# gregorgebhardt/gym-kilobots

Hardware: AMD Instinct MI355X
Metric: kilobot-steps/sec (higher is better)
Workload: dtype f32

## Files before the change

gym_kilobots_amd/csrc/kb_regsolve_bins.inc:

```
{
    constexpr int KRB = KB_KREG_BINS;
    const bool solving = (int)__builtin_amdgcn_readfirstlane(wave) < nsolve;
    unsigned ra[KRB], rb[KRB], rm[KRB];
    float racc[KRB], rnx[KRB], rny[KRB];
    const unsigned WOFF = 8u * (unsigned)(NB - 5);
    char *const velB = reinterpret_cast<char *>(vel), *const posB = reinterpret_cast<char *>(pos);
#define RB_WALL(j) (ra[j] >= WOFF)
#define RB_WALLIDX(j) ((int)((ra[j] - WOFF) >> 3))
#define RB_VEL(off) (*reinterpret_cast<float2 *>(velB + (off)))
#define RB_POS(off) (*reinterpret_cast<float2 *>(posB + (off)))
#define RB_C(j) ((int)(rm[j] & 0xFFFu))
#define RB_DEPTH(j) ((int)((rm[j] >> 12) & 0x1FFu))
#define RB_FLIP(j) (((rm[j] >> 21) & 1u) != 0u)
#define RB_ISL(j) ((int)(rm[j] >> 22))
#pragma unroll
    for (int j = 0; j < KRB; ++j) { ra[j] = 0u; rb[j] = 0u; rm[j] = 0u; racc[j] = 0.0f; rnx[j] = 1.0f; rny[j] = 0.0f; }
    unsigned long long slotLevels[KRB];
    int dlo[KRB], dhi[KRB];
#pragma unroll
    for (int j = 0; j < KRB; ++j) { slotLevels[j] = 0ull; dlo[j] = 1; dhi[j] = 0; }
    int maxD = 0;
    unsigned mycnt = 0;
    const float nm_bb = p.nm_bb, nm_wb = p.nm_wb;
#ifdef KB_SOLVER_PRIO
// ... 173 lines not shown
                ra[j] = wallA ? WOFF + 8u * (unsigned)(a - WALL_CODE) : 8u * (unsigned)a;
                rb[j] = 8u * (unsigned)b;
                racc[j] = v_[j] ? acc_[j] : 0.0f;
                rm[j] = v_[j] ? (c_[j] | ((unsigned)rdepth[j] << 12) | (flip ? 1u << 21 : 0u) | (root_[j] << 22)) : 0u;
                float dist;
                wall_geom(p, wallA ? a - WALL_CODE : 0, pb_[j].x, pb_[j].y, dist, wnx[j], wny[j]);
                if (flip) { wnx[j] = -wnx[j]; wny[j] = -wny[j]; }
                dx[j] = pb_[j].x - pa_[j].x; dy[j] = pb_[j].y - pa_[j].y;
                dd[j] = dx[j] * dx[j] + dy[j] * dy[j];
                pairOn[j] = v_[j] && !wallA && dd[j] > B2_EPSILON * B2_EPSILON;
                ieee = ieee || (pairOn[j] && !kb_exact_guard(dd[j]));
                if (wallA) { rnx[j] = wnx[j]; rny[j] = wny[j]; } else { rnx[j] = 1.0f; rny[j] = 0.0f; }
            }
            if (__builtin_expect(__builtin_amdgcn_ballot_w64(ieee) == 0ull, 1)) {
#pragma unroll
                for (int j = 0; j < KRB; ++j) {
                    const float len = kb_sqrt_refine(dd[j], __builtin_amdgcn_sqrtf(dd[j]), __builtin_amdgcn_rsqf(dd[j]));
                    const float inv = kb_rcp_refine(len, __builtin_amdgcn_rcpf(len));
                    if (pairOn[j]) { rnx[j] = dx[j] * inv; rny[j] = dy[j] * inv; }
                }
            } else {
#pragma unroll
                for (int j = 0; j < KRB; ++j) {
                    const float len = sqrtf(dd[j]);
                    const float inv = 1.0f / len;
                    if (pairOn[j]) { rnx[j] = dx[j] * inv; rny[j] = dy[j] * inv; }
                }
            }
        }
#undef RB_A
#undef RB_B
#ifdef KB_PROFILE
        if (lane == 0) atomicMax(&misc[M_PROF], (unsigned)maxD);
        if (tid == 0) atomicAdd(&KB_PROF(M_PROF_DEPTH), (unsigned)maxD);
        KB_STAMP(7);
#endif
    }
    KB_ABLATE_EXIT(9);
#define RB_ON(j) (RB_DEPTH(j) == d_)
    if (solving) {
#pragma unroll
        for (int j = 0; j < KRB; ++j) {
            for (int d_ = dlo[j]; d_ <= dhi[j]; ++d_) {
                if (RB_ON(j)) {
                    const float2 va = RB_VEL(ra[j]), vb = RB_VEL(rb[j]);
                    const float Px = racc[j] * rnx[j], Py = racc[j] * rny[j];
                    const float ima = RB_WALL(j) ? 0.0f : p.im_bot;
                    RB_VEL(ra[j]) = make_float2(va.x - ima * Px, va.y - ima * Py);
                    RB_VEL(rb[j]) = make_float2(vb.x + p.im_bot * Px, vb.y + p.im_bot * Py);
                }
                wave_sync();
            }
        }
        KB_STAMP_PRE(29);
    }
    KB_ABLATE_EXIT(10);
    if (solving) {
        for (int it = 0; it < p.vel_iters; ++it) {
#pragma unroll
            for (int j = 0; j < KRB; ++j) {
                for (int d_ = dlo[j]; d_ <= dhi[j]; ++d_) {
                    if (RB_ON(j)) {
                        const float2 va = RB_VEL(ra[j]), vb = RB_VEL(rb[j]);
                        const bool wallA = RB_WALL(j);
                        const float nx = rnx[j], ny = rny[j];
                        const float ima = wallA ? 0.0f : p.im_bot, imb = p.im_bot;
                        const float dvx = vb.x - va.x, dvy = vb.y - va.y;
                        const float vn = dvx * nx + dvy * ny;
                        float lambda = -((wallA ? nm_wb : nm_bb) * vn);
                        const float accOld = racc[j];
                        const float newimp = fmaxf(accOld + lambda, 0.0f);
                        lambda = newimp - accOld;
                        racc[j] = newimp;
                        const float Px = lambda * nx, Py = lambda * ny;
                        RB_VEL(ra[j]) = make_float2(va.x - ima * Px, va.y - ima * Py);
                        RB_VEL(rb[j]) = make_float2(vb.x + imb * Px, vb.y + imb * Py);
                    }
                    wave_sync();
                }
            }
        }
        KB_STAMP_PRE(30);
    }
#ifdef KB_SOLVER_PRIO
    __builtin_amdgcn_s_setprio(0);
#endif
    __syncthreads();
    KB_STAMP(4);
    KB_RETID();
    KB_ABLATE_EXIT(11);
#ifdef KB_PROFILE
    if (tid == 0) atomicAdd(&KB_PROF(9), misc[M_PROF]);
#endif
    if (solving) {
#pragma unroll
        for (int j = 0; j < KRB; ++j)
            if (lane + 64u * j < mycnt) lAcc[RB_C(j)] = racc[j];
    }
#pragma unroll
    for (int q = 0; q < BPT; ++q) {
        const int b_ = tid + q * nt;
        if (b_ >= N) continue;
        const int b = ms[q];
        float vxx = vel[b].x, vyy = vel[b].y, ww = bw[q];
        startX[b] = pos[b].x; startY[b] = pos[b].y;
        const float tx = h * vxx, ty = h * vyy;
        if (tx * tx + ty * ty > B2_MAX_TRANSLATION_SQ) {
            const float ratio = B2_MAX_TRANSLATION / sqrtf(tx * tx + ty * ty);
            vxx *= ratio; vyy *= ratio;
        }
        const float rot = h * ww;
        if (rot * rot > B2_MAX_ROTATION_SQ) {
            const float ratio = B2_MAX_ROTATION / fabsf(rot);
            ww *= ratio;
        }
        pos[b].x += h * vxx; pos[b].y += h * vyy;
        th[q] += h * ww;
        vel[b].x = vxx; vel[b].y = vyy; bw[q] = ww;
        if (SLEEP) islWave[b] = (unsigned char)((active[b] ? 2 : 0) | (p.pos_iters <= 0 ? 1 : 0));
    }
    __syncthreads();
    KB_STAMP(5);
    KB_RETID();
    KB_ABLATE_EXIT(12);
    if (solving) {
#ifdef KB_SOLVER_PRIO
        __builtin_amdgcn_s_setprio(KB_SOLVER_PRIO);
#endif
        for (int it = 0; it < p.pos_iters; ++it) {
            unsigned char *act = active + (it & 1) * NB, *nxt = active + ((it + 1) & 1) * NB;
            bool viol = false;
            bool ron[KRB];
#pragma unroll
            for (int j = 0; j < KRB; ++j) ron[j] = (lane + 64u * j < mycnt) && act[RB_ISL(j)] != 0;
#pragma unroll
            for (int j = 0; j < KRB; ++j) {
                for (int d_ = dlo[j]; d_ <= dhi[j]; ++d_) {
                    if (ron[j] && RB_ON(j)) {
                    const bool wallA = RB_WALL(j);
                    const int isl = RB_ISL(j);
                    float nx, ny, sep;
                    const float ima = wallA ? 0.0f : p.im_bot, imb = p.im_bot;
                    const float2 pb = RB_POS(rb[j]);
                    const float bx = pb.x, by = pb.y;
                    float axx = 0.0f, ayy = 0.0f;
                    if (wallA) {
                        float dist, wx, wy;
                        wall_geom(p, RB_WALLIDX(j), bx, by, dist, wx, wy);
                        nx = RB_FLIP(j) ? -wx : wx; ny = RB_FLIP(j) ? -wy : wy;
                        const float along = RB_FLIP(j) ? -dist : dist;
                        sep = along - B2_POLYGON_RADIUS - p.r_bot;
                    } else {
                        const float2 pa = RB_POS(ra[j]);
                        axx = pa.x; ayy = pa.y;
                        const float dx = bx - axx, dy = by - ayy;
                        const float dd = dx * dx + dy * dy;
                        if (__builtin_expect(__builtin_amdgcn_ballot_w64(!kb_exact_guard(dd)) == 0ull, 1)) {
                            const float len = kb_sqrt_refine(dd, __builtin_amdgcn_sqrtf(dd), __builtin_amdgcn_rsqf(dd));
                            const float inv = kb_rcp_refine(len, __builtin_amdgcn_rcpf(len));
                            nx = dx * inv; ny = dy * inv;
                        } else {
                            const float len = sqrtf(dd);
                            nx = dx; ny = dy;
                            if (!(len < B2_EPSILON)) { const float inv = 1.0f / len; nx = dx * inv; ny = dy * inv; }
                        }
                        sep = (dx * nx + dy * ny) - p.r_bot - p.r_bot;
                    }
                    if (sep < -3.0f * B2_LINEAR_SLOP) { nxt[isl] = 1; viol = true; if (SLEEP && it == p.pos_iters - 1) islWave[isl] = 3; }
                    const float C = kb_clampf(B2_BAUMGARTE * (sep + B2_LINEAR_SLOP), -B2_MAX_LINEAR_CORRECTION, 0.0f);
                    const float K = ima + imb;
                    const float imp = __builtin_expect(p.exact_div, 1) ? kb_div_const(-C, K, wallA ? p.y_wb : p.y_bb) : (K > 0.0f ? -C / K : 0.0f);
                    const float Px = imp * nx, Py = imp * ny;
                    if (!wallA) RB_POS(ra[j]) = make_float2(axx - ima * Px, ayy - ima * Py);
                    RB_POS(rb[j]) = make_float2(bx + imb * Px, by + imb * Py);
                    }
                    wave_sync();
                }
            }
#ifdef KB_PROFILE
            if (tid == 0) atomicAdd(&KB_PROF(10), 1u);
#endif
            if (!__any(viol)) break;
#pragma unroll
            for (int j = 0; j < KRB; ++j) if (lane + 64u * j < mycnt) act[RB_ISL(j)] = 0;
            wave_sync();
        }
        KB_STAMP_PRE(24);
#ifdef KB_SOLVER_PRIO
        __builtin_amdgcn_s_setprio(0);
#endif
    }
#undef RB_WALL
#undef RB_WALLIDX
#undef RB_VEL
#undef RB_POS
#undef RB_C
#undef RB_DEPTH
#undef RB_FLIP
#undef RB_ISL
#undef RB_ON
}
```

gym_kilobots_amd/csrc/kb_step_kernel.h:

```cpp
#pragma once
#include <utility>

#include "kb_common.h"
#include "kb_objects.h"

namespace kb {

template <int DRIVE_MODE, int LIGHT_TYPE, bool OBJ, int FN = 0, int TIER = 0, bool POLY = true, bool SENSE = true, bool SLEEP = false>
__global__ void __launch_bounds__(TIER == 1 ? 64 : 64 * KB_MAX_WAVES, (TIER == 1 || TIER == 3) ? 2 : ((TIER == 2 || (FN != 0 && !OBJ)) ? KB_COMPACT_WAVES_PER_SIMD : KB_MIN_WAVES_PER_SIMD)) kb_step_kernel(const Params p) {
    constexpr bool WIDE = TIER == 1 || TIER == 3;
    constexpr bool BINS = !OBJ;
    constexpr int KRX = BINS ? KB_KREG_BINS : KREG;
    constexpr bool PAR_DS = FN != 0 && BINS;
    static_assert(!SLEEP || FN == 0 || !OBJ, "the fixed-size instantiations with objects do not carry the sleep state");
    extern __shared__ __align__(16) unsigned char smem[];
    int e = blockIdx.x;
    int tid = threadIdx.x;
    const int nt = FN ? 64 * KB_MAX_WAVES : (int)blockDim.x;
    int lane = tid & 63, wave = tid >> 6;
    const int wave_s = __builtin_amdgcn_readfirstlane(wave);
    const int nw = nt >> 6;
    const int nsolve = BINS ? (nw >= KB_NSOLVE_DIV ? nw / KB_NSOLVE_DIV : 1) : nw;
    const int N = FN ? FN : p.N, NP = FN ? ((FN + 3) & ~3) : p.NP, S = p.S;
    size_t o = (size_t)e * N;
    size_t wo = (size_t)e * p.cap;
    const float h = p.h;

    const int NB = FN ? ((FN + 3) & ~3) + KB_MAX_OBJECTS + 4 : p.NB;
    const int capL_ = (BINS && FN != 0) ? ldsb::CAPL : p.capL;
    const bool hashed = FN == 0 && p.hmask != 0;
    const int fx = lds::fixed(OBJ || FN != 0, nw), ot_ = lds::objtab(nw);
    float2 *pos = (float2 *)(smem + (BINS ? ldsb::pos() : lds::body32(fx, NB, 0))), *vel = (float2 *)(smem + (BINS ? ldsb::vel(NB) : lds::body32(fx, NB, 2)));
    float2 *start = (float2 *)(smem + lds::body32(fx, NB, 4));
    unsigned *dirCnt = (unsigned *)(smem + (BINS ? ldsb::dircnt(NB) : lds::body32(fx, NB, 6))), *parent = (unsigned *)(smem + (BINS ? ldsb::parent(NB) : lds::body32(fx, NB, 7)));
    unsigned *islCnt = dirCnt;
    unsigned *lPair = (unsigned *)(smem + (BINS ? ldsb::con32(NB, NP, hashed, capL_, 0) : lds::con32(fx, NB, capL_, 0))), *lInfo = (unsigned *)(smem + (BINS ? ldsb::con32(NB, NP, hashed, capL_, 1) : lds::con32(fx, NB, capL_, 1)));
    float *lAcc = (float *)(smem + (BINS ? ldsb::con32(NB, NP, hashed, capL_, 2) : lds::con32(fx, NB, capL_, 2)));
    float *oldAcc = (float *)(smem + (BINS ? ldsb::oldacc(NB, NP, hashed, capL_) : lds::con32(fx, NB, capL_, 3)));
    unsigned short *lCbk = (unsigned short *)(smem + (BINS ? ldsb::cbk(NB, NP, hashed, capL_) : lds::con16(fx, NB, capL_, 0)));
    unsigned short *lOrder = (unsigned short *)(smem + (BINS ? ldsb::order(NB, NP, hashed, capL_) : lds::con16(fx, NB, capL_, 1)));
    unsigned short *oldKey = (unsigned short *)(smem + (BINS ? ldsb::oldkey(NB, NP, hashed, capL_) : lds::con16(fx, NB, capL_, 2)));
    unsigned short *wsOff = (unsigned short *)(smem + (BINS ? ldsb::wsoff(NB) : lds::bot16(fx, NB, capL_, NP, 0))), *newOff = (unsigned short *)(smem + (BINS ? ldsb::newoff(NB, NP, hashed) : lds::bot16(fx, NB, capL_, NP, 1)));
    unsigned short *nextb = (unsigned short *)(smem + lds::bot16(fx, NB, capL_, NP, 2)), *cellOf = (unsigned short *)(smem + lds::bot16(fx, NB, capL_, NP, 3));
    unsigned char *wsCnt = smem + (BINS ? ldsb::wscnt(NB, NP) : lds::bot8(fx, NB, capL_, NP, 0)), *wsCntNew = smem + (BINS ? ldsb::wscntnew(NB, NP, hashed) : lds::bot8(fx, NB, capL_, NP, 1));
    unsigned char *active = smem + (BINS ? ldsb::act0(NB, NP, hashed, capL_) : lds::active(fx, NB, capL_, NP));
    unsigned char *islWave = smem + (BINS ? ldsb::islwave(NB, NP, hashed, capL_) : lds::islwave(fx, NB, capL_, NP));
    unsigned short *head = (unsigned short *)(smem + lds::head(fx, NB, capL_, NP));
    unsigned short *idOf = (unsigned short *)(smem + ldsb::idof(NB, NP)), *cellOfSlot = (unsigned short *)(smem + ldsb::cellofslot(NB, NP));
    unsigned short *E1 = (unsigned short *)(smem + ldsb::binE(NB, NP, hashed, capL_));
    unsigned short *tmpSort = reinterpret_cast<unsigned short *>(lInfo);
    float *startX = reinterpret_cast<float *>(smem + ldsb::botA(NB)), *startY = reinterpret_cast<float *>(dirCnt);
    unsigned *misc = (unsigned *)(smem + lds::MISC), *wsum = (unsigned *)(smem + lds::WSUM);
    const int tb_ = BINS ? ldsb::binE(NB, NP, hashed, capL_) - lds::BKSTART : 0;
    unsigned *bkStart = (unsigned *)(smem + tb_ + lds::BKSTART), *bkFill = (unsigned *)(smem + tb_ + lds::bkfill(nw));
    unsigned *bkMaxRank = (unsigned *)(smem + tb_ + lds::bkmaxrank(nw));
    unsigned short *bkList = (unsigned short *)(smem + tb_ + lds::bklist(nw));
    unsigned char *nList = smem + tb_ + lds::nlist(nw);
    float *objTab = (float *)(smem + ot_);
    float *objBody = (float *)(smem + ot_ + lds::OBJBODY);
    unsigned *objCnt = (unsigned *)(smem + ot_ + lds::OBJCNT);
    unsigned short *objList = (unsigned short *)(smem + ot_ + lds::OBJLIST);
    float *objW = (float *)(smem + ot_ + lds::OBJW), *objA = (float *)(smem + ot_ + lds::OBJA), *objA0 = (float *)(smem + ot_ + lds::OBJA0);
    unsigned long long *mcMask = (unsigned long long *)(smem + ot_ + lds::MCMASK);
    float *objSlp = (float *)(smem + ot_ + lds::OBJSLP);
    const int M = OBJ ? p.M : 0;
    constexpr bool MIX = DRIVE_MODE == KB_DRIVE_MIXED;
    static_assert(!MIX || (OBJ && FN == 0), "mixed drive laws run on the generic code path with per-body masses");
    unsigned char *botLaw = smem + (MIX ? p.botlaw_off : 0);
#define KB_IM_BOT(a_) (MIX ? p.im_mode[botLaw[a_]] : p.im_bot)
    auto bim = [&](int id) __attribute__((always_inline)) -> float {
        return id >= WALL_CODE ? 0.0f : ((!OBJ || id < N) ? KB_IM_BOT(id) : objBody[(id - N) * BT_WORDS + BT_IM]);
    };
    auto brad = [&](int id) __attribute__((always_inline)) -> float {
        return id >= WALL_CODE ? B2_POLYGON_RADIUS : ((!OBJ || id < N) ? p.r_bot : objBody[(id - N) * BT_WORDS + BT_RADIUS]);
    };
    auto bpoly = [&](int id) __attribute__((always_inline)) -> bool {
        return OBJ && POLY && id >= N && id < WALL_CODE && objBody[(id - N) * BT_WORDS + BT_KIND] != 0.0f;
    };
    ObjCtx ox;
    ox.pos = pos; ox.vel = vel; ox.objW = objW; ox.objA = objA; ox.objTab = objTab; ox.objBody = objBody;
    ox.mc = (float *)(smem + lds::mcarea(fx, NB, capL_, NP, p.nhead));
    ox.N = N; ox.MCN = p.nmc; ox.mu_oo = p.mu_oo; ox.mu_ow = p.mu_ow;
    const int NMC = OBJ ? p.nmc : 0;
    const int F = OBJ ? p.F : 0;

    const kb_buffers &g = p.buf;
    auto hix = [&](int cell_) __attribute__((always_inline)) -> int { return hashed ? (cell_ & p.hmask) : cell_; };
    unsigned *gPair, *gInfo;
    float *gAcc;
    unsigned short *gCbk, *gOrder;
#define KB_ENV_ADDRESSES()                                                                          \
    do {                                                                                            \
        int e_ = blockIdx.x;                                                                        \
        asm volatile("" : "+s"(e_));                                                                \
        e = e_; o = (size_t)e * N; wo = (size_t)e * p.cap;                                          \
        gPair = reinterpret_cast<unsigned *>(g.scratch) + wo * 4;                                   \
        gInfo = gPair + p.cap;                                                                      \
        gAcc = reinterpret_cast<float *>(gInfo + p.cap);                                            \
        gCbk = reinterpret_cast<unsigned short *>(gAcc + p.cap); gOrder = gCbk + p.cap;             \
    } while (0)
    KB_ENV_ADDRESSES();

#ifdef KB_PROFILE
    static_assert(M_COUNT <= 24, "profile words start at misc[24]");
    constexpr int M_PROF_DEPTH = 12;
    if (tid < 40) misc[24 + tid] = 0;
    __syncthreads();
    unsigned prof_t = (unsigned)clock64();
#endif

    float th[BPT], bw[BPT], cv[BPT], cw[BPT], av[BPT], aw[BPT];
    float sth0[BPT];
    float slp[BPT];
    int law[BPT];
    int ms[BPT];
#define KB_LAW(q) (MIX ? law[q] : DRIVE_MODE)
    constexpr bool PARK = BINS && !MIX && DRIVE_MODE == KB_DRIVE_VELOCITY;
#define KB_SLOT(q, b_) (BINS ? ms[q] : (b_))
    float ldx[BPT], ldy[BPT];
    unsigned ldc[BPT];
    float2 lda[BPT];
#pragma unroll
    for (int q = 0; q < BPT; ++q) {
        const int b = tid + q * nt;
        th[q] = 0.0f; bw[q] = 0.0f; cv[q] = 0.0f; cw[q] = 0.0f; av[q] = 0.0f; aw[q] = 0.0f; slp[q] = 0.0f; law[q] = DRIVE_MODE;
        float z_ = 0.0f;
        asm volatile("" : "+v"(z_));
        ldx[q] = 0.0f; ldy[q] = 0.0f; ldc[q] = 0u; lda[q] = make_float2(z_, z_);
        ms[q] = b < N ? b : NB - 1;
        if (b < N) {
            ldx[q] = g.x[o + b]; ldy[q] = g.y[o + b]; th[q] = g.theta[o + b];
            if (MIX) law[q] = min((int)g.bot_mode[o + b], 4);
            if (SLEEP) slp[q] = g.sleep_time[o + b];
            ldc[q] = g.ws_cnt[o + b];
            const bool velmode = KB_LAW(q) == KB_DRIVE_VELOCITY || KB_LAW(q) == KB_DRIVE_ACCEL;
            if (velmode && !(KB_LAW(q) == KB_DRIVE_VELOCITY && p.actions)) { cv[q] = g.v[o + b]; cw[q] = g.w[o + b]; }
            if (KB_LAW(q) == KB_DRIVE_ACCEL) { av[q] = g.acc_v[o + b]; aw[q] = g.acc_w[o + b]; }
            if (p.actions && velmode) lda[q] = reinterpret_cast<const float2 *>(p.actions)[o + b];
        }
    }
// ... 1052 lines not shown
        auto mc_velocity_pass = [&](unsigned long long mask, bool leader) __attribute__((always_inline)) {
            if (leader) for (unsigned long long m_ = mask; m_; m_ &= m_ - 1) mc_solve_velocity(ox, __builtin_ctzll(m_));
        };
        auto mc_position_pass = [&](unsigned long long mask, bool leader, const unsigned char *act, unsigned char *nxt, bool lastIt) __attribute__((always_inline)) -> bool {
            bool viol = false;
            if (leader)
                for (unsigned long long m_ = mask; m_; m_ &= m_ - 1) {
                    const int t = __builtin_ctzll(m_);
                    const int isl = mci(ox, MC_ISL, t);
                    if (!act[isl]) continue;
                    const float minSep = mc_solve_position(ox, t, B2_BAUMGARTE);
                    if (minSep < -3.0f * B2_LINEAR_SLOP) { nxt[isl] = 1; viol = true; if (SLEEP && lastIt) islWave[isl] = 3; }
                }
            return viol;
        };
        auto mc_clear_flags = [&](unsigned long long mask, bool leader, unsigned char *act) __attribute__((always_inline)) {
            if (leader) for (unsigned long long m_ = mask; m_; m_ &= m_ - 1) act[mci(ox, MC_ISL, __builtin_ctzll(m_))] = 0;
        };
        auto mc_store = [&]() __attribute__((always_inline)) {
            if (OBJ && wave == 0 && lane < NMC) {
                int owner, col;
                mc_candidate(F, lane, owner, col);
                float *dst = owsMine + (owner * KB_OWS_COLS + col) * KB_OWS_WORDS;
                float o[KB_OWS_WORDS] = {-1.0f, -1.0f, -1.0f, -1.0f, -1.0f, -1.0f};
                if (mcTouch) {
                    const int cnt = (mci(ox, MC_TYPE, lane) >> 2) & 3, ids = mci(ox, MC_ID, lane);
                    o[0] = (float)(ids & 255); o[1] = mcf(ox, MC_NI0, lane); o[2] = mcf(ox, MC_TI0, lane);
                    if (cnt == 2) { o[3] = (float)((ids >> 8) & 255); o[4] = mcf(ox, MC_NI1, lane); o[5] = mcf(ox, MC_TI1, lane); }
                }
#pragma unroll
                for (int k = 0; k < KB_OWS_WORDS; ++k) dst[k] = o[k];
            }
        };
        auto bucket_sort = [&](const unsigned *sPair, const unsigned *sInfo, unsigned short *cbk,
                               unsigned short *order) __attribute__((always_inline)) {
            const int W = coop ? 1 : nw;
            for (int b = tid; b < N + M; b += nt) islCnt[b] = 0;
            for (int k = tid; k < W * BK_PER_WAVE; k += nt) { bkStart[k] = 0; bkFill[k] = 0; }
            for (int k = tid; k < W * NUM_CLS; k += nt) bkMaxRank[k] = 0;
            if (tid == 0) bkStart[W * BK_PER_WAVE] = 0;
            __syncthreads();
            for (int c = tid; c < ncon; c += nt) {
                const unsigned root = parent[sPair[c] >> 16];
                if (SLEEP && !active[root]) { cbk[c] = EMPTY16; continue; }
                const int w = coop ? 0 : (int)islWave[root];
                const unsigned inf = sInfo[c];
                const int cls = inf & 0x7F, r = (inf >> 8) & 0xFF;
                const int bk = (w * NUM_CLS + cls) * RK + (r < RK - 1 ? r : RK - 1);
                cbk[c] = (unsigned short)bk;
                atomicAdd(&bkStart[bk], 1u);
                if (r >= RK - 1) atomicMax(&bkMaxRank[w * NUM_CLS + cls], (unsigned)r);
            }
            __syncthreads();
            if (wave == 0) {
                const int nb = W * BK_PER_WAVE;
                const int chunk = (nb + 63) / 64;
                const int s0 = lane * chunk, e0 = min(nb, s0 + chunk);
                unsigned sum = 0;
                for (int i = s0; i < e0; ++i) sum += bkStart[i];
                const unsigned incl = wave_incl_scan(sum);
                unsigned run = incl - sum;
                for (int i = s0; i < e0; ++i) { unsigned v = bkStart[i]; bkStart[i] = run; run += v; }
                if (lane == 63) bkStart[nb] = incl;
            }
            __syncthreads();
            for (int c = tid; c < ncon; c += nt) {
                const int bk = cbk[c];
                if (SLEEP && bk == (int)EMPTY16) continue;
                order[bkStart[bk] + atomicAdd(&bkFill[bk], 1u)] = (unsigned short)c;
            }
            if (wave < W) {
                const int base = wave * BK_PER_WAVE;
                const bool ne = lane < BK_PER_WAVE && bkStart[base + lane + 1] > bkStart[base + lane];
                const unsigned long long m = __ballot(ne);
                if (ne) bkList[base + __popcll(m & ((1ull << lane) - 1ull))] = (unsigned short)(base + lane);
                if (lane == 0) nList[wave] = (unsigned char)__popcll(m);
            }
            __syncthreads();
        };
        if (reg) {
            for (int b = tid; b < N + M; b += nt) islCnt[b] = 0;
            if (tid < nw * NUM_CLS) bkMaxRank[tid] = 0;
            if constexpr (BINS) {
                if (wave_s == 0) {
                    const unsigned v_ = lane < nw ? misc[M_WCNT + lane] : 0u;
                    const unsigned incl = wave_incl_scan(v_);
                    if (lane < nw) misc[M_WFILL + lane] = incl - v_;
                }
                __syncthreads();
                for (int c = tid; c < ncon; c += nt) {
                    const unsigned w = islWave[parent[lPair[c] >> 16]];
                    lOrder[atomicAdd(&misc[M_WFILL + w], 1u)] = (unsigned short)c;
                }
            } else {
                for (int c = tid; c < ncon; c += nt) {
                    const unsigned w = islWave[parent[lPair[c] >> 16]];
                    unsigned base = 0;
                    for (unsigned w2 = 0; w2 < w; ++w2) base += misc[M_WCNT + w2];
                    lOrder[base + atomicAdd(&misc[M_WFILL + w], 1u)] = (unsigned short)c;
                }
            }
            __syncthreads();
        } else if (big) bucket_sort(gPair, gInfo, gCbk, gOrder);
        else bucket_sort(lPair, lInfo, lCbk, lOrder);
        KB_STAMP(3);
        KB_RETID();
        KB_ABLATE_EXIT(8);

        const bool coopLevels = BINS && coopForced && nw > 1;
        if constexpr (BINS) {
            if (reg) {
#include "kb_regsolve_bins.inc"
            } else if (coopLevels) {
#include "kb_coopsolve_bins.inc"
            }
        }
        if (BINS && (reg || coopLevels)) {
        } else if (reg) {
            unsigned mybase = 0;
            for (int w = 0; w < wave; ++w) mybase += misc[M_WCNT + w];
            const unsigned mycnt = misc[M_WCNT + wave];
            int ra[KREG], rb[KREG], rkey[KREG], rrank[KREG], rslot[KREG], risl[KREG], rc[KREG], rdepth[KREG];
            float racc[KREG], rnx[KREG], rny[KREG], rima[KREG], rimb[KREG], rra[KREG], rrb[KREG], rnm[KREG];
            bool rvalid[KREG], rflip[KREG];
            bool rpoly[KREG];
            float rrAx[KREG], rrAy[KREG], rlnx[KREG], rlny[KREG], rlpx[KREG], rlpy[KREG];
            unsigned mlo = 0, mhi = 0;
            const float nm_bb = p.nm_bb, nm_wb = p.nm_wb;
#define R_IMA(j) (OBJ ? rima[j] : (ra[j] < WALL_CODE ? p.im_bot : 0.0f))
#define R_IMB(j) (OBJ ? rimb[j] : p.im_bot)
#define R_RA(j) (OBJ ? rra[j] : (ra[j] < WALL_CODE ? p.r_bot : B2_POLYGON_RADIUS))
#define R_RB(j) (OBJ ? rrb[j] : p.r_bot)
#define R_NM(j) (OBJ ? rnm[j] : (ra[j] < WALL_CODE ? nm_bb : nm_wb))
#pragma unroll
            for (int j = 0; j < KREG; ++j) {
                const unsigned idx = lane + 64u * j;
                rvalid[j] = idx < mycnt;
                ra[j] = 0; rb[j] = 0; rkey[j] = 0; rrank[j] = 0; rc[j] = 0; rdepth[j] = 0;
                if (rvalid[j]) {
                    const int c = lOrder[mybase + idx];
                    const unsigned pr = lPair[c], inf = lInfo[c];
                    const int cls = inf & 0x7F, r = (inf >> 8) & 0xFF;
                    rc[j] = c; ra[j] = pr & 0xFFFF; rb[j] = pr >> 16; rrank[j] = r;
                    const int key = cls * RK + (r < RK - 1 ? r : RK - 1);
                    if (SLEEP && !active[parent[rb[j]]]) {
                        rkey[j] = -1;
                    } else {
                        rkey[j] = key;
                        if (key < 32) mlo |= 1u << key; else mhi |= 1u << (key - 32);
                        if (r >= RK - 1) atomicMax(&bkMaxRank[wave * NUM_CLS + cls], (unsigned)r);
                    }
                }
            }
            mlo = wave_or(mlo); mhi = wave_or(mhi);
            const unsigned long long keymask = ((unsigned long long)mhi << 32) | mlo;
            wave_sync();
#ifdef KB_PROFILE
            if (tid == 0) { atomicAdd(&KB_PROF(8), (unsigned)__popcll(keymask)); atomicAdd(&KB_PROF(11), 1u); }
#endif

#define KB_REG_KEY_ROUNDS(...)                                                                      \
            for (unsigned long long m_ = keymask; m_; m_ &= m_ - 1) {                               \
                const int key_ = __builtin_ctzll(m_);                                               \
                if ((key_ % RK) < RK - 1) {                                                         \
                    _Pragma("unroll") for (int j = 0; j < KREG; ++j)                                \
                        if (rvalid[j] && rkey[j] == key_) { __VA_ARGS__ }                           \
                    wave_sync();                                                                    \
                } else {                                                                            \
                    const int maxr_ = (int)bkMaxRank[wave * NUM_CLS + key_ / RK];                   \
                    for (int r_ = RK - 1; r_ <= maxr_; ++r_) {                                      \
                        _Pragma("unroll") for (int j = 0; j < KREG; ++j)                            \
                            if (rvalid[j] && rkey[j] == key_ && rrank[j] == r_) { __VA_ARGS__ }     \
                        wave_sync();                                                                \
                    }                                                                               \
                }                                                                                   \
// ... 655 lines not shown
                            const int m = b - N;
                            const float *T = objTab + ((KB_INF >> 24) & 15u) * OT_WORDS;
                            V2 ln, lp;
                            collide_poly_circle(T, xf_of_body(objBody + m * BT_WORDS, start[b].x, start[b].y, objA0[m]), mk2(start[a].x, start[a].y), p.r_bot, ln, lp);
                            const XF xo = body_xf(ox, b);
                            const V2 normal = rot_mul(xo, ln);
                            const V2 planePoint = xf_mul(xo, lp);
                            const V2 clipPoint = mk2(pos[a].x, pos[a].y);
                            const float sep = v_dot(v_sub(clipPoint, planePoint), normal) - T[OT_RADIUS] - p.r_bot;
                            const V2 rA = v_sub(clipPoint, mk2(pos[b].x, pos[b].y));
                            if (sep < -3.0f * B2_LINEAR_SLOP) { nxt[isl] = 1; viol = true; if (SLEEP && it == p.pos_iters - 1) islWave[isl] = 3; }
                            const float C = kb_clampf(B2_BAUMGARTE * (sep + B2_LINEAR_SLOP), -B2_MAX_LINEAR_CORRECTION, 0.0f);
                            const float rnA = v_cross(rA, normal);
                            const float K = T[OT_IM] + KB_IM_BOT(a) + T[OT_II] * rnA * rnA;
                            const float imp = K > 0.0f ? -C / K : 0.0f;
                            const V2 P = v_scale(imp, normal);
                            pos[b].x -= T[OT_IM] * P.x; pos[b].y -= T[OT_IM] * P.y;
                            objA[m] -= T[OT_II] * v_cross(rA, P);
                            pos[a].x += KB_IM_BOT(a) * P.x; pos[a].y += KB_IM_BOT(a) * P.y;
                        } else if (act[isl]) {
                            float nx, ny, sep;
                            const float ima = bim(a), imb = bim(b), rda = brad(a), rdb = brad(b);
                            const float bx = pos[b].x, by = pos[b].y;
                            float axx = 0.0f, ayy = 0.0f;
                            if (a >= WALL_CODE) {
                                float dist, wx, wy;
                                wall_geom(p, a - WALL_CODE, bx, by, dist, wx, wy);
                                const bool flipped = (KB_INF & 0x80) != 0;
                                nx = flipped ? -wx : wx; ny = flipped ? -wy : wy;
                                const float along = flipped ? -dist : dist;
                                sep = along - rda - rdb;
                            } else {
                                axx = pos[a].x; ayy = pos[a].y;
                                const float dx = bx - axx, dy = by - ayy;
                                const float len = sqrtf(dx * dx + dy * dy);
                                nx = dx; ny = dy;
                                if (!(len < B2_EPSILON)) { const float inv = 1.0f / len; nx = dx * inv; ny = dy * inv; }
                                sep = (dx * nx + dy * ny) - rda - rdb;
                            }
                            if (sep < -3.0f * B2_LINEAR_SLOP) { nxt[isl] = 1; viol = true; if (SLEEP && it == p.pos_iters - 1) islWave[isl] = 3; }
                            const float C = kb_clampf(B2_BAUMGARTE * (sep + B2_LINEAR_SLOP), -B2_MAX_LINEAR_CORRECTION, 0.0f);
                            const float K = ima + imb;
                            const float imp = K > 0.0f ? -C / K : 0.0f;
                            const float Px = imp * nx, Py = imp * ny;
                            if (a < WALL_CODE) { pos[a].x = axx - ima * Px; pos[a].y = ayy - ima * Py; }
                            pos[b].x = bx + imb * Px; pos[b].y = by + imb * Py;
                        }
                    })
                    if (OBJ && myMc) { viol |= mc_position_pass(myMc, leader, act, nxt, it == p.pos_iters - 1); KB_ROUND_SYNC(); }
#ifdef KB_PROFILE
                    if (tid == 0) atomicAdd(&KB_PROF(10), 1u);
#endif
                    bool any;
                    if (coop) {
                        if (viol) misc[M_ANY] = 1u;
                        __syncthreads();
                        any = misc[M_ANY] != 0u;
                        __syncthreads();
                        if (tid == 0) misc[M_ANY] = 0u;
                    } else {
                        any = __any(viol);
                    }
                    if (!any) break;
                    {
                        const int s_ = (int)bkStart[myw * BK_PER_WAVE], e_ = (int)bkStart[(myw + 1) * BK_PER_WAVE];
                        for (int i_ = s_ + lid; i_ < e_; i_ += stride) act[parent[sPair[order[i_]] >> 16]] = 0;
                        if (OBJ && myMc) mc_clear_flags(myMc, leader, act);
                    }
                    KB_ROUND_SYNC();
                }
#undef KB_FOR_ROUNDS
#undef KB_FOR_ROUNDS_PF
#undef KB_FOR_ROUNDS_PLAIN
#undef KB_VEL_NORMAL
#undef KB_ROUND_SYNC
            };
            if (big) {
                float *gN = reinterpret_cast<float *>(g.scratch) + (size_t)p.E * p.cap * 4 + wo * 3;
                solve_list(gPair, gInfo, gAcc, gCbk, gOrder, gN, true);
            } else solve_list(lPair, lInfo, lAcc, lCbk, lOrder, nullptr, false);
        }
        __syncthreads();
        KB_STAMP_PRE(25);
        KB_RETID();
        KB_ABLATE_EXIT(13);
        if (SLEEP) {
            unsigned *islMin = BINS ? reinterpret_cast<unsigned *>(smem + (FN ? ldsb::binE(NB, NP, false, capL_) : p.islmin_off)) : lPair;
            const float linTolSqr = B2_LINEAR_SLEEP_TOL * B2_LINEAR_SLEEP_TOL, angTolSqr = B2_ANGULAR_SLEEP_TOL * B2_ANGULAR_SLEEP_TOL;
            for (int b = tid; b < N + M; b += nt) islMin[b] = 0x7F7FFFFFu;
            __syncthreads();
#pragma unroll
            for (int q = 0; q < BPT; ++q) {
                const int b_ = tid + q * nt;
                if (b_ >= N) continue;
                const int b = KB_SLOT(q, b_);
                const unsigned r = parent[b];
                if (!(islWave[r] & 2)) continue;
                if (slp[q] < 0.0f) slp[q] = 0.0f;
                const float2 v_ = vel[b];
                if (bw[q] * bw[q] > angTolSqr || v_.x * v_.x + v_.y * v_.y > linTolSqr) { slp[q] = 0.0f; atomicMin(&islMin[r], 0u); }
                else { slp[q] += h; atomicMin(&islMin[r], __float_as_uint(slp[q])); }
            }
            if (tid < M) {
                const int b = N + tid;
                const unsigned r = parent[b];
                if (islWave[r] & 2) {
                    float sl = objSlp[tid];
                    if (sl < 0.0f) sl = 0.0f;
                    const float2 v_ = vel[b];
                    const float w_ = objW[tid];
                    if (w_ * w_ > angTolSqr || v_.x * v_.x + v_.y * v_.y > linTolSqr) { sl = 0.0f; atomicMin(&islMin[r], 0u); }
                    else { sl += h; atomicMin(&islMin[r], __float_as_uint(sl)); }
                    objSlp[tid] = sl;
                }
            }
            __syncthreads();
#pragma unroll
            for (int q = 0; q < BPT; ++q) {
                const int b_ = tid + q * nt;
                if (b_ >= N) continue;
                const int b = KB_SLOT(q, b_);
                const unsigned r = parent[b];
                const unsigned st_ = islWave[r];
                if ((st_ & 2) && !(st_ & 1) && __uint_as_float(islMin[r]) >= B2_TIME_TO_SLEEP) {
                    slp[q] = -1.0f; vel[b].x = 0.0f; vel[b].y = 0.0f; bw[q] = 0.0f;
                }
            }
            if (tid < M) {
                const int b = N + tid;
                const unsigned r = parent[b];
                const unsigned st_ = islWave[r];
                if ((st_ & 2) && !(st_ & 1) && __uint_as_float(islMin[r]) >= B2_TIME_TO_SLEEP) {
                    objSlp[tid] = -1.0f; vel[b].x = 0.0f; vel[b].y = 0.0f; objW[tid] = 0.0f;
                }
            }
            __syncthreads();
        }
        bool toiRecords = false;
        if (p.toi_walls) {
            float *cTh0 = reinterpret_cast<float *>(BINS ? parent : lInfo), *cTh = BINS ? reinterpret_cast<float *>(lPair) : lAcc;
            float *cW = reinterpret_cast<float *>(BINS ? lOrder : lCbk);
            unsigned short *cSlot = reinterpret_cast<unsigned short *>(active);
            const int candMax = BINS ? min(capL_, N) : capL_ / 2;
            int cand[BPT];
            if (!BINS) {
                if (tid == 0) misc[M_NCON] = 0;
                __syncthreads();
            }
#pragma unroll
            for (int q = 0; q < BPT; ++q) {
                const int b_ = tid + q * nt;
                cand[q] = -1;
                if (b_ >= N) continue;
                const int b = KB_SLOT(q, b_);
                if (SLEEP && slp[q] < 0.0f) continue;
                const float xa = BINS ? startX[b] : start[b].x, ya = BINS ? startY[b] : start[b].y, xb = pos[b].x, yb = pos[b].y;
                bool none = true;
#pragma unroll
                for (int wl = 0; wl < 4; ++wl) none &= kb_toi_no_event(p, wl, p.toi_tt, xa, ya, xb, yb);
                if (none) continue;
                const int i = (int)atomicAdd(&misc[M_NCON], 1u);
                if (i >= candMax) { atomicOr(&misc[M_STATUS], 8u); continue; }
                cand[q] = i;
                if (BINS) cSlot[i] = (unsigned short)b; else lPair[i] = (unsigned)b;
                cTh0[i] = sth0[q]; cTh[i] = th[q]; cW[i] = bw[q];
            }
// ... 134 lines not shown
```

Baseline: 16.75 billion.

## Integrate contact bodies in solver waves to drop block barriers around integration

Replaces the block-wide integration loop, which sat between two __syncthreads, with per-wave integration. Each solver wave integrates the bodies of its own contacts, chosen where the body's depth matches the slot depth. A new LDS bitmask (intMark, aliased onto bkList) marks bodies touched by any contact so owner threads integrate only the unconstrained ones, and only wave_sync is needed. This removes two block barriers and lets position iterations start without waiting for other waves. It relies on depth-based ownership being exclusive and on bkList being free to alias, which is a correctness risk.

```diff
diff --git a/gym_kilobots_amd/csrc/kb_regsolve_bins.inc b/gym_kilobots_amd/csrc/kb_regsolve_bins.inc
--- a/gym_kilobots_amd/csrc/kb_regsolve_bins.inc
+++ b/gym_kilobots_amd/csrc/kb_regsolve_bins.inc
@@ -279,51 +279,86 @@
         }
         KB_STAMP_PRE(30);
     }
-#ifdef KB_SOLVER_PRIO
-    __builtin_amdgcn_s_setprio(0);
-#endif
-    __syncthreads();
     KB_STAMP(4);
     KB_RETID();
     KB_ABLATE_EXIT(11);
-#ifdef KB_PROFILE
-    if (tid == 0) atomicAdd(&KB_PROF(9), misc[M_PROF]);
-#endif
     if (solving) {
 #pragma unroll
         for (int j = 0; j < KRB; ++j)
             if (lane + 64u * j < mycnt) lAcc[RB_C(j)] = racc[j];
     }
-#pragma unroll
-    for (int q = 0; q < BPT; ++q) {
-        const int b_ = tid + q * nt;
-        if (b_ >= N) continue;
-        const int b = ms[q];
-        float vxx = vel[b].x, vyy = vel[b].y, ww = bw[q];
-        startX[b] = pos[b].x; startY[b] = pos[b].y;
-        const float tx = h * vxx, ty = h * vyy;
-        if (tx * tx + ty * ty > B2_MAX_TRANSLATION_SQ) {
-            const float ratio = B2_MAX_TRANSLATION / sqrtf(tx * tx + ty * ty);
-            vxx *= ratio; vyy *= ratio;
-        }
-        const float rot = h * ww;
-        if (rot * rot > B2_MAX_ROTATION_SQ) {
-            const float ratio = B2_MAX_ROTATION / fabsf(rot);
-            ww *= ratio;
-        }
-        pos[b].x += h * vxx; pos[b].y += h * vyy;
-        th[q] += h * ww;
-        vel[b].x = vxx; vel[b].y = vyy; bw[q] = ww;
-        if (SLEEP) islWave[b] = (unsigned char)((active[b] ? 2 : 0) | (p.pos_iters <= 0 ? 1 : 0));
-    }
-    __syncthreads();
+    {
+        const unsigned char unsolved = (unsigned char)(p.pos_iters <= 0 ? 1 : 0);
+        char *const sxB = reinterpret_cast<char *>(startX), *const syB = reinterpret_cast<char *>(startY);
+        auto integrate_xy = [&](const unsigned off8, const float2 v0, const float2 p0) __attribute__((always_inline)) {
+            float vxx = v0.x, vyy = v0.y;
+            *reinterpret_cast<float *>(sxB + (off8 >> 1)) = p0.x; *reinterpret_cast<float *>(syB + (off8 >> 1)) = p0.y;
+            const float tx = h * vxx, ty = h * vyy;
+            if (tx * tx + ty * ty > B2_MAX_TRANSLATION_SQ) {
+                const float ratio = B2_MAX_TRANSLATION / sqrtf(tx * tx + ty * ty);
+                vxx *= ratio; vyy *= ratio;
+            }
+            RB_POS(off8) = make_float2(p0.x + h * vxx, p0.y + h * vyy);
+            RB_VEL(off8) = make_float2(vxx, vyy);
+        };
+        bool intA[KRB], intB[KRB], own[BPT];
+        {
+            unsigned dA[KRB], dB[KRB], mk[BPT];
+            const char *const bdB = reinterpret_cast<const char *>(islCnt);
+#pragma unroll
+            for (int j = 0; j < KRB; ++j) {
+                dA[j] = *reinterpret_cast<const unsigned *>(bdB + ((RB_WALL(j) ? rb[j] : ra[j]) >> 1));
+                dB[j] = *reinterpret_cast<const unsigned *>(bdB + (rb[j] >> 1));
+            }
+#pragma unroll
+            for (int q = 0; q < BPT; ++q) mk[q] = intMark[(unsigned)ms[q] & 31u];
+#pragma unroll
+            for (int j = 0; j < KRB; ++j) {
+                const unsigned d = (unsigned)RB_DEPTH(j);
+                intA[j] = solving && d != 0u && !RB_WALL(j) && dA[j] == d;
+                intB[j] = solving && d != 0u && dB[j] == d;
+            }
+#pragma unroll
+            for (int q = 0; q < BPT; ++q) {
+                own[q] = tid + q * nt < N && ((mk[q] >> ((unsigned)ms[q] >> 5)) & 1u) == 0u;
+            }
+        }
+        wave_sync();
+        static_assert(KRB == BPT, "a register slot and a kilobot of the owner thread share a trip");
+#pragma unroll
+        for (int j = 0; j < KRB; ++j) {
+            const unsigned oo = 8u * (unsigned)ms[j];
+            const float2 vO = RB_VEL(oo), pO = RB_POS(oo);
+            const unsigned char aO = SLEEP ? active[ms[j]] : (unsigned char)1;
+            if (j == 0 || mycnt > 64u) {
+                const float2 vA = RB_VEL(ra[j]), vB = RB_VEL(rb[j]), pA = RB_POS(ra[j]), pB = RB_POS(rb[j]);
+                if (intA[j]) {
+                    integrate_xy(ra[j], vA, pA);
+                    if (SLEEP) islWave[ra[j] >> 3] = (unsigned char)(2 | unsolved);
+                }
+                if (intB[j]) {
+                    integrate_xy(rb[j], vB, pB);
+                    if (SLEEP) islWave[rb[j] >> 3] = (unsigned char)(2 | unsolved);
+                }
+            }
+            if (own[j]) {
+                integrate_xy(oo, vO, pO);
+                if (SLEEP) islWave[ms[j]] = (unsigned char)((aO ? 2 : 0) | unsolved);
+            }
+            float ww = bw[j];
+            const float rot = h * ww;
+            if (rot * rot > B2_MAX_ROTATION_SQ) {
+                const float ratio = B2_MAX_ROTATION / fabsf(rot);
+                ww *= ratio;
+            }
+            th[j] += h * ww;
+            bw[j] = ww;
+        }
+    }
+    wave_sync();
     KB_STAMP(5);
-    KB_RETID();
     KB_ABLATE_EXIT(12);
     if (solving) {
-#ifdef KB_SOLVER_PRIO
-        __builtin_amdgcn_s_setprio(KB_SOLVER_PRIO);
-#endif
         for (int it = 0; it < p.pos_iters; ++it) {
             unsigned char *act = active + (it & 1) * NB, *nxt = active + ((it + 1) & 1) * NB;
             bool viol = false;
@@ -383,10 +418,10 @@
             wave_sync();
         }
         KB_STAMP_PRE(24);
+    }
 #ifdef KB_SOLVER_PRIO
-        __builtin_amdgcn_s_setprio(0);
+    __builtin_amdgcn_s_setprio(0);
 #endif
-    }
 #undef RB_WALL
 #undef RB_WALLIDX
 #undef RB_VEL
diff --git a/gym_kilobots_amd/csrc/kb_step_kernel.h b/gym_kilobots_amd/csrc/kb_step_kernel.h
--- a/gym_kilobots_amd/csrc/kb_step_kernel.h
+++ b/gym_kilobots_amd/csrc/kb_step_kernel.h
@@ -56,6 +56,8 @@
     unsigned *bkMaxRank = (unsigned *)(smem + tb_ + lds::bkmaxrank(nw));
     unsigned short *bkList = (unsigned short *)(smem + tb_ + lds::bklist(nw));
     unsigned char *nList = smem + tb_ + lds::nlist(nw);
+    unsigned *intMark = reinterpret_cast<unsigned *>(bkList);
+    static_assert(BPT * 64 * KB_MAX_WAVES <= 1024 && lds::nbk(1) >= 64, "32 words of intMark hold a bit for every slot");
     float *objTab = (float *)(smem + ot_);
     float *objBody = (float *)(smem + ot_ + lds::OBJBODY);
     unsigned *objCnt = (unsigned *)(smem + ot_ + lds::OBJCNT);
@@ -1274,6 +1276,7 @@
             for (int b = tid; b < N + M; b += nt) islCnt[b] = 0;
             if (tid < nw * NUM_CLS) bkMaxRank[tid] = 0;
             if constexpr (BINS) {
+                if (tid < 32) intMark[tid] = 0;
                 if (wave_s == 0) {
                     const unsigned v_ = lane < nw ? misc[M_WCNT + lane] : 0u;
                     const unsigned incl = wave_incl_scan(v_);
@@ -1281,8 +1284,14 @@
                 }
                 __syncthreads();
                 for (int c = tid; c < ncon; c += nt) {
-                    const unsigned w = islWave[parent[lPair[c] >> 16]];
+                    const unsigned pr = lPair[c], a = pr & 0xFFFFu, b = pr >> 16;
+                    const unsigned root = parent[b];
+                    const unsigned w = islWave[root];
                     lOrder[atomicAdd(&misc[M_WFILL + w], 1u)] = (unsigned short)c;
+                    if (!SLEEP || active[root] != 0) {
+                        atomicOr(&intMark[b & 31u], 1u << (b >> 5));
+                        if (a < (unsigned)WALL_CODE) atomicOr(&intMark[a & 31u], 1u << (a >> 5));
+                    }
                 }
             } else {
                 for (int c = tid; c < ncon; c += nt) {
@@ -2104,6 +2113,9 @@
         }
         __syncthreads();
         KB_STAMP_PRE(25);
+#ifdef KB_PROFILE
+        if (BINS && reg && tid == 0) atomicAdd(&KB_PROF(9), misc[M_PROF]);
+#endif
         KB_RETID();
         KB_ABLATE_EXIT(13);
         if (SLEEP) {
```

Result: faster. 16.96 billion, median of 6 (+1.2%).
